# rafaelcgon/2D-GP

Measured on AMD Instinct MI355X. Metric: posterior grid points/sec (fit+predict), N_train=4096, div-free 2D kernel, higher is better.
Workload: dtype f64 (variance GEMM as exact int8 Ozaki-II); 1 GPU; df kernel, N_train=4096, 256x256 grid per GPU, fit+predict (mean+variance); n_train=4096, grid_per_gpu=256x256, points_total=65536, parallelism=grid-sharded x1, factor local, kstar_ahead=False

## Files before the change

2d-gp_amd/csrc/gp2d.hip:

```cpp
#include "common.hpp"
#ifndef GP2D_RELEASE
#error "libgp2d.so is built with -DGP2D_RELEASE=1 (python __graft_entry__.py build)"
#endif
#include "assemble.hpp"
#include "gemm_f64.hpp"
#include "factor.hpp"
#include "predict.hpp"
#include "fields.hpp"
#include "grad.hpp"
#include "postcov.hpp"
#include "predict_host.hpp"
#include "ozaki.hpp"
#include "ozaki_host.hpp"
#include "factor_host.hpp"
#include "lml.hpp"
#include "lml_host.hpp"
#include "dfact.hpp"
#include "order.hpp"
#include "../../include/gp2d.h"

#include <dlfcn.h>

#include <algorithm>
#include <cstdlib>
// ... 1044 lines not shown
  p.diag_add = diag_add;
  p.C = cov; p.ldc = ldc;
  TimedLaunch t(s, 2.0 * (double)ntr * (double)(2 * m) * (double)(2 * m));
  return launch_postcov(p, s);
}

int gp2d_ozaki_nmod(int64_t n) { return ozaki_nmod_for(n); }

size_t gp2d_ozaki_wres_bytes(int64_t n) {
  const int nm = ozaki_nmod_for(n);
  return nm > 0 ? (size_t)nm * (size_t)n * (size_t)n : 0;
}

static int launch_w_res(const double* W, int64_t n, WRows ldw, const OzakiConsts& oc, int8_t* wres,
                        const double* rowscale, hipStream_t s) {
  ozaki_w_res_kernel<<<dim3((unsigned)(n / 64), (unsigned)(n / 256)), 256, 0, s>>>(W, n, ldw, oc, wres, rowscale);
  return check_launch("ozaki_w_res_kernel");
}

static int prepare_args(const gp2d_kernel_t* k, int wbits, int kbits, int64_t n, bool bufs_ok, const int* nmod_out) {
  GP2D_CHECK(validate_ozaki_kernel(k));
  GP2D_CHECK(valid_bits(wbits, kbits));
  GP2D_REQUIRE(n % IBM == 0 && n > 0, "ozaki: n must be a positive multiple of 256");
  GP2D_REQUIRE(bufs_ok, "ozaki: NULL buffer");
  GP2D_REQUIRE(nmod_out != nullptr, "ozaki: nmod_out is NULL");
  return 0;
}

static int prepare_finish(int nmod, const gp2d_kernel_t* k, int pw, int pb, const double* W, int64_t n, WRows wr,
                          int8_t* wres, double* rowscale, bool fused, int* nmod_out, hipStream_t s) {
  OzakiConsts oc;
// ... 105 lines not shown
      const double e = gp2d_ozaki_error_model(kss, vmin, pw, pb);
      if (e <= target && e < best) { best = e; bw = pw; bk = pb; }
    }
    if (bw) {
      *wbits = bw;
      *kbits = bk;
      return 1;
    }
  }
  return 0;
}

static int g_oz_skip = 1;
void gp2d_ozaki_set_skip(int on) { g_oz_skip = on ? 1 : 0; }

size_t gp2d_predict_ozaki_workspace(int64_t n, int64_t chunk) {
  return OzakiWork(n, chunk, ozaki_nmod_for(n), true).total;
}

size_t gp2d_predict_ozaki_workspace_nmod(int64_t n, int64_t chunk, int nmod) {
  if (nmod <= 0 || nmod > ozaki_nmod_for(n)) return 0;
  return std::max(OzakiWork(n, chunk, nmod, true).total, OzakiWork(n, chunk, nmod, false).total);
}

size_t gp2d_predict_ozaki_planes_workspace(int64_t n, int64_t chunk) {
  return OzakiWork(n, chunk, ozaki_nmod_for(n), false).total;
}

struct OzakiChunk {
  int64_t cv, cp, ncols;
  const double* xg;
  dim3 kgrid;
  OzakiChunk(const double* xg0, int64_t m, int64_t c0, int64_t chunk, int64_t ntr_pad, const gp2d_kernel_t* k)
      : cv(std::min<int64_t>(chunk, m - c0)), cp(round_up(cv, IBN)), ncols(2 * cp), xg(xg0 + point_dim(k) * c0),
        kgrid((unsigned)((ntr_pad + OZ_KS_T - 1) / OZ_KS_T), (unsigned)(cp / OZ_KS_P)) {}
};

static int launch_kstar(const OzakiChunk& c, hipStream_t s, const double* xtr, int64_t ntr, int64_t npad,
                        const VecParams& vp, const double* alpha, const OzakiConsts& oc, int8_t* bres, double* pm,
                        uint8_t* flags) {
  if ((uint64_t)(2 * npad) * (uint64_t)c.ncols < (1ull << 31))
    ozaki_kstar_kernel<true><<<c.kgrid, 256, 0, s>>>(xtr, ntr, npad, c.xg, c.cv, c.cp, vp, alpha, oc, bres, pm, flags);
  else
    ozaki_kstar_kernel<false><<<c.kgrid, 256, 0, s>>>(xtr, ntr, npad, c.xg, c.cv, c.cp, vp, alpha, oc, bres, pm, flags);
  return check_launch("ozaki_kstar_kernel");
}

static int predict_ozaki_impl(const int8_t* wres, const double* rowscale, int nmod, int kbits, int64_t n,
                              const double* alpha, const double* xtr, int64_t ntr,
                              int64_t ntr_pad, const double* xg, int64_t m, const gp2d_kernel_t* k, int var_mode,
                              double noise, int compute_var, double* mean, double* var,
                              const int64_t* out_order, int64_t chunk, const OzakiWork& lay, void* work,
                              const KstarBuf* pre, const int8_t* pre_base, hipStream_t s) {
  const auto [bres, cres, pm, P, flags, skip] = lay.at(work);
  OzakiConsts oc;
  GP2D_CHECK(make_ozaki_consts(nmod, k, oc, OZ_PW, ozaki_kbits(kbits)));
  const int nm = oc.nmod;
  GP2D_REQUIRE(n < 131072, "ozaki: the int8 GEMM epilogue needs n < 131072 (N_train < 65536)");
  const int64_t nmseg = (ntr_pad + OZ_KS_T - 1) / OZ_KS_T;
// ... 13 lines not shown
    const size_t bplane = (size_t)ncols * n;
    const bool inline_planes = compute_var && !pre;
    GP2D_CHECK(launch_kstar(c, s, xtr, ntr, ntr_pad, vp, alpha, inline_planes ? oc : oc_mean_only,
                            pre ? nullptr : bres, pm, inline_planes ? flags : nullptr));
    const int nbj = (int)(ncols / IBN), kslabs = (int)(n / IBK);
    const bool use_skip = compute_var && g_oz_skip && kslabs <= (1 << 20);
    int* slist = skip;
    int* scnt = skip + (int64_t)nbj * kslabs;
    if (use_skip) {
      ozaki_slab_list_kernel<<<(unsigned)nbj, 64, 0, s>>>(F, (int)(ntr_pad / OZ_KS_T), nbj, kslabs, slist, scnt);
      GP2D_CHECK(check_launch("ozaki_slab_list_kernel"));
    }
    if (compute_var) {
      const double nv = 2.0 * (double)ntr;
      TimedLaunch timed(s, 2.0 * (double)cv * nv * nv);
      const int zper = (n <= kIgemmZBatchMaxN) ? nm : 1;
      for (int l0 = 0; l0 < nm; l0 += zper) {
        const int nz = std::min(zper, nm - l0);
        IgemmZ zb{(int64_t)n * n, (int64_t)bplane, (int64_t)n * ncols, {}};
        for (int u = 0; u < nz; ++u) zb.m[u] = oc.m[l0 + u];
        constexpr int tbn = 256, nst = I_NSTAGE;
        const dim3 ggrid((unsigned)(ncols / tbn), (unsigned)(n / IBM), (unsigned)nz);
        const int8_t* Al = wres + (size_t)l0 * n * n;
        const int8_t* Bl = B + (size_t)l0 * bplane;
        uint8_t* Cl = cres + (size_t)l0 * n * ncols;
        igemm_nt_mod_kernel<tbn, nst><<<ggrid, 2 * tbn, 0, s>>>(Al, Bl, Cl, n, (int)n, (int)ncols, (int)n, 1, oc.m[l0],
                                                                (int)(cp / IBN), (int)(ntr_pad / IBK),
                                                                use_skip ? slist : nullptr, use_skip ? scnt : nullptr,
                                                                zb);
        GP2D_CHECK(check_launch("igemm_nt_mod_kernel"));
      }
      timed.stop();
      const dim3 cgrid((unsigned)((ncols + OZ_CRT_BCOLS - 1) / OZ_CRT_BCOLS), (unsigned)npseg);
      ozaki_crt_colsq_kernel<<<cgrid, 256, 0, s>>>(cres, n, ncols, oc, rowscale, P);
      GP2D_CHECK(check_launch("ozaki_crt_colsq_kernel"));
    }
    GP2D_CHECK(launch_finalize({pm, nmseg, P, npseg, ncols, cp, cv, c0, m, kss, add, clip, compute_var, mean, var,
                                out_order}, s));
  }
  return 0;
}

static int predict_ozaki_args(const gp2d_kernel_t* k, int64_t n, int64_t ntr_pad, int64_t chunk, int var_mode,
                              bool ptrs_ok, int64_t m, int nmod, int kbits, const OzakiWork& lay, const void* work,
                              size_t work_bytes) {
// ... 503 lines not shown
```

2d-gp_amd/csrc/ozaki.hpp:

```cpp
#pragma once
#include <type_traits>
#include "common.hpp"
#include "assemble.hpp"

namespace gp2d {

constexpr int OZ_MAXMOD = 20;
#ifdef GP2D_OZ_P
#define GP2D_OZ_PW GP2D_OZ_P
#define GP2D_OZ_PB GP2D_OZ_P
#endif
#ifndef GP2D_OZ_PW
#define GP2D_OZ_PW 49
#endif
#ifndef GP2D_OZ_PB
#define GP2D_OZ_PB 45
#endif
constexpr int OZ_PW = GP2D_OZ_PW;
constexpr int OZ_PB = GP2D_OZ_PB;
static_assert(OZ_PW <= 50 && OZ_PB <= 50, "ozaki: the one-part residues need |x| < 2^50");
constexpr int OZ_PW_MAX = 60;
constexpr int OZ_PB_MAX = 50;
constexpr int OZ_SPLIT = 26;
constexpr int OZ_HBITS = 33;
// ... 68 lines not shown
    rowscale[i] = final_scale ? ldexp(M, -si - sB) : (double)si;
    if (l1 != nullptr) l1[i] = sum;
  }
}

__global__ __launch_bounds__(256) void ozaki_rowscale_final_kernel(double* __restrict__ rowscale, int64_t n, double M,
                                                                   int sB) {
  const int64_t i = (int64_t)blockIdx.x * 256 + threadIdx.x;
  if (i < n) rowscale[i] = ldexp(M, -(int)rowscale[i] - sB);
}

__device__ __forceinline__ int ozaki_row_exp(double rowscale_i, const OzakiConsts& oc) {
  return ilogb(oc.M) - ilogb(rowscale_i) - oc.sB;
}

__global__ __launch_bounds__(256) void ozaki_w_res_kernel(const double* __restrict__ W, int64_t n, WRows wr,
                                                          OzakiConsts oc, int8_t* __restrict__ wres,
                                                          const double* __restrict__ rowscale) {
  const int64_t bi = blockIdx.y, ks = blockIdx.x;
  if (ks * 64 >= (bi + 1) * 256) return;
  const int lane = threadIdx.x & 63, wv = threadIdx.x >> 6;
  const int64_t k0 = ks * 64 + 4 * (lane & 15);
  const int64_t plane = n * n;
#pragma unroll 1
  for (int it = 0; it < 16; ++it) {
    const int64_t i = bi * 256 + wv * 64 + it * 4 + (lane >> 4);
    const int si = ozaki_row_exp(rowscale[i], oc);
    const double* w = W + wr.off(i) + k0;
    d2 p0 = {0.0, 0.0}, p1 = {0.0, 0.0};
    if (k0 < wr.len(i, n)) {
      p0 = *reinterpret_cast<const d2*>(w);
      p1 = *reinterpret_cast<const d2*>(w + 2);
    }
    const double v[4] = {p0.x, p0.y, p1.x, p1.y};
    double x[4], xm[4];
#pragma unroll
    for (int u = 0; u < 4; ++u) {
      x[u] = (k0 + u <= i) ? rint(ldexp(v[u], si)) : 0.0;
      xm[u] = x[u] + OZ_MAGIC52;
    }
    int8_t* dst = wres + slab_offset(i, k0, n);
    if (oc.pw <= 50) {
      for (int l = 0; l < oc.nmod; ++l) {
        const double m = oc.md[l], im = oc.inv_m[l];
        uint32_t r[4];
#pragma unroll
        for (int u = 0; u < 4; ++u) r[u] = residue_low_m(x[u], xm[u], m, im);
        *reinterpret_cast<uint32_t*>(dst + (int64_t)l * plane) = pack22(pack2_lo(r[0], r[1]), pack2_lo(r[2], r[3]));
      }
    } else {
      double xh[4], xl[4];
#pragma unroll
      for (int u = 0; u < 4; ++u) {
        xh[u] = rint(ldexp(x[u], -OZ_SPLIT));
        xl[u] = x[u] - ldexp(xh[u], OZ_SPLIT);
      }
      for (int l = 0; l < oc.nmod; ++l) {
        const double m = oc.md[l], im = oc.inv_m[l], c = oc.c26[l];
        uint32_t r[4];
#pragma unroll
        for (int u = 0; u < 4; ++u) {
          const double rh = fma(-m, rint(xh[u] * im), xh[u]), rl = fma(-m, rint(xl[u] * im), xl[u]);
          const double t = fma(rh, c, rl);
          r[u] = residue_low_m(t, t + OZ_MAGIC52, m, im);
        }
        *reinterpret_cast<uint32_t*>(dst + (int64_t)l * plane) = pack22(pack2_lo(r[0], r[1]), pack2_lo(r[2], r[3]));
      }
    }
  }
}

#ifndef GP2D_KS_OCC
#define GP2D_KS_OCC 5
#endif
#ifndef GP2D_KS_PPL
#define GP2D_KS_PPL 2
#endif
constexpr int OZ_KS_T = 64;
constexpr int OZ_KS_P = 64;
constexpr int OZ_KS_PPL = GP2D_KS_PPL;
static_assert(OZ_KS_PPL == 2 || OZ_KS_PPL == 4, "2 or 4 training points per lane");

template <int PPL> struct packed_bytes;
template <> struct packed_bytes<2> { typedef uint16_t type; };
template <> struct packed_bytes<4> { typedef uint32_t type; };

template <bool OFF32>
__global__ __launch_bounds__(256, GP2D_KS_OCC) void ozaki_kstar_kernel(
    const double* __restrict__ xtr, int64_t ntr, int64_t npad, const double* __restrict__ xg, int64_t cv,
    int64_t cp, VecParams vp, const double* __restrict__ alpha, OzakiConsts oc, int8_t* __restrict__ bres,
    double* __restrict__ pm, uint8_t* __restrict__ flags) {
  constexpr int PPL = OZ_KS_PPL, LG = 64 / PPL, RPW = 64 / LG, RPI = 4 * RPW;
  typedef typename packed_bytes<PPL>::type pk_t;
  const int lane = threadIdx.x & 63, wv = threadIdx.x >> 6;
  const int kg = lane % LG, r = lane / LG;
  const int64_t t0 = (int64_t)blockIdx.x * OZ_KS_T + PPL * kg;
  const int64_t n = 2 * npad, ncols = 2 * cp;
  double a1[PPL], a2[PPL], x0[PPL], x1[PPL], x2[PPL];
  bool tv[PPL];
#pragma unroll
  for (int u = 0; u < PPL; ++u) {
    const int64_t t = t0 + u;
// ... 29 lines not shown
        mu += __shfl_xor(mu, o);
        mv += __shfl_xor(mv, o);
      }
      if (kg == 0 && p < cp) {
        pm[(int64_t)blockIdx.x * ncols + p] = mu;
        pm[(int64_t)blockIdx.x * ncols + cp + p] = mv;
      }
    }
    if (p >= cp || t0 >= npad) continue;
    double xi[3][PPL], xm[3][PPL];
#pragma unroll
    for (int u = 0; u < PPL; ++u) {
      xi[0][u] = rint(k11[u] * scale);
      xi[1][u] = rint(k12[u] * scale);
      xi[2][u] = rint(k22[u] * scale);
      nz = nz || xi[0][u] != 0.0 || xi[1][u] != 0.0 || xi[2][u] != 0.0;
#pragma unroll
      for (int e = 0; e < 3; ++e) xm[e][u] = xi[e][u] + OZ_MAGIC52;
    }
    const int64_t o_uu = slab_offset(p, t0, n), o_uv = slab_offset(p, npad + t0, n),
                  o_vv = slab_offset(cp + p, npad + t0, n);
    const int64_t pstride = ncols * n;
    for (int l = 0; l < oc.nmod; ++l) {
      const double m = oc.md[l], im = oc.inv_m[l];
      pk_t pk[3];
#pragma unroll
      for (int e = 0; e < 3; ++e) {
        uint32_t r[PPL];
#pragma unroll
        for (int u = 0; u < PPL; ++u) r[u] = residue_low_m(xi[e][u], xm[e][u], m, im);
        if constexpr (PPL == 2) pk[e] = (pk_t)pack2_lo(r[0], r[1]);
        else pk[e] = (pk_t)pack22(pack2_lo(r[0], r[1]), pack2_lo(r[2], r[3]));
      }
      int8_t* plane = bres + (int64_t)l * pstride;
      if constexpr (OFF32) {
        const __amdgpu_buffer_rsrc_t rs = __builtin_amdgcn_make_buffer_rsrc(plane, (short)0, (int)pstride, 0x00020000);
        if constexpr (PPL == 2) {
          __builtin_amdgcn_raw_buffer_store_b16(pk[0], rs, (int)o_uu, 0, 0);
          __builtin_amdgcn_raw_buffer_store_b16(pk[1], rs, (int)o_uv, 0, 0);
          __builtin_amdgcn_raw_buffer_store_b16(pk[2], rs, (int)o_vv, 0, 0);
        } else {
          __builtin_amdgcn_raw_buffer_store_b32(pk[0], rs, (int)o_uu, 0, 0);
          __builtin_amdgcn_raw_buffer_store_b32(pk[1], rs, (int)o_uv, 0, 0);
          __builtin_amdgcn_raw_buffer_store_b32(pk[2], rs, (int)o_vv, 0, 0);
        }
      } else {
        *reinterpret_cast<pk_t*>(plane + o_uu) = pk[0];
// ... 72 lines not shown
#endif
}

__device__ __forceinline__ int swz16(int row, int chunk) {
  const int q = (row >> 2) & 3;
  const int g = (0x78 >> (2 * q)) & 3;
  return chunk ^ g;
}

template <int P, int W>
__device__ __forceinline__ void vmwait_barrier(std::integral_constant<int, W>) {
  static_assert(P * W < 64, "vmcnt field");
  asm volatile("s_waitcnt vmcnt(%0)\n\ts_waitcnt lgkmcnt(0)\n\ts_barrier" ::"n"(P * W) : "memory");
}

struct IgemmZ {
  int64_t sA, sB, sC;
  int m[OZ_MAXMOD];
};
constexpr int64_t kIgemmZBatchMaxN = 4096;

template <int TBN, int NST>
__global__ __launch_bounds__(TBN * 2, (TBN == 256) ? 1 : 2) void igemm_nt_mod_kernel(
    const int8_t* __restrict__ A, const int8_t* __restrict__ B, uint8_t* __restrict__ C, int64_t ldc, int M, int N,
    int K, int a_lower, int modulus, int alias_rb, int alias_ks, const int* __restrict__ slist,
    const int* __restrict__ scnt, const IgemmZ zb) {
  if (gridDim.z > 1) {
    A += blockIdx.z * zb.sA;
    B += blockIdx.z * zb.sB;
    C += blockIdx.z * zb.sC;
    modulus = zb.m[blockIdx.z];
  }
  static_assert(TBN == 256 || TBN == 128, "tile width");
  static_assert(NST >= 3 && NST <= 5, "ring depth 3..5 (the tail is written out for these)");
  constexpr int NW = TBN / 32;
  constexpr int WC = TBN / 64;
  constexpr int B_OP = TBN * IBK;
  constexpr int STG = I_OP + B_OP;
  constexpr int AP = IBM / NW / 16;
  constexpr int BPW = TBN / NW / 16;
  constexpr int PPW = AP + BPW;
  __shared__ __attribute__((aligned(16))) int8_t smem[NST * STG];
  const int bj = blockIdx.x;
  const int bi = (int)(gridDim.y - 1 - blockIdx.y);
  const int i0 = bi * IBM, j0 = bj * TBN;
  const int jb = j0 / IBN, jr = j0 % IBN;
  const int ke = a_lower ? min(K, i0 + IBM) : K;
  const int tid = threadIdx.x, lane = tid & 63, wid = __builtin_amdgcn_readfirstlane(tid >> 6);
  const int wr = wid / WC, wc = wid % WC;
  const int l16 = lane & 15, lq = lane >> 4;
  const int64_t kslabs = K / IBK;
  const int8_t* Ap = A + (int64_t)bi * kslabs * I_OP;
  const bool alias = jb >= alias_rb;
  const int8_t* Bp = B + (int64_t)jb * kslabs * I_OP + jr * IBK;
  const int8_t* Bq = B + ((int64_t)(alias ? jb - alias_rb : 0) * kslabs + alias_ks) * I_OP + jr * IBK;
  int nsl = ke / IBK;
  const int* sl = nullptr;
  if (slist != nullptr) {
    const int c = scnt[(int64_t)jb * (kslabs / 4 + 1) + ke / IBM];
    if (c == 0 || c >= NST - 1) {
      nsl = c;
      sl = slist + (int64_t)jb * kslabs;
    }
  }

  const int bias = (int)ozaki_acc_bias(K, modulus);
  i4v acc[8][4];
#pragma unroll
  for (int mi = 0; mi < 8; ++mi)
#pragma unroll
    for (int ni = 0; ni < 4; ++ni) acc[mi][ni] = i4v{bias, bias, bias, bias};

  const int drow = lane >> 2, dchunk = lane & 3;
  const int rec = (int)(kslabs * I_OP);
  const __amdgpu_buffer_rsrc_t rA = __builtin_amdgcn_make_buffer_rsrc((void*)Ap, (short)0, rec, 0x00020000);
  const __amdgpu_buffer_rsrc_t rBp = __builtin_amdgcn_make_buffer_rsrc((void*)Bp, (short)0, rec, 0x00020000);
  const __amdgpu_buffer_rsrc_t rBq = __builtin_amdgcn_make_buffer_rsrc((void*)Bq, (short)0, rec, 0x00020000);
  int voA[AP], voB[BPW];
#pragma unroll
  for (int h = 0; h < AP; ++h) {
    const int row = (wid * AP + h) * 16 + drow;
    voA[h] = row * IBK + 16 * swz16(row, dchunk);
  }
#pragma unroll
  for (int h = 0; h < BPW; ++h) {
    const int row = (wid * BPW + h) * 16 + drow;
    voB[h] = row * IBK + 16 * swz16(jr + row, dchunk);
  }
  auto issue = [&](int ks, int st) {
    int8_t* As = smem + st * STG;
    int8_t* Bs = As + I_OP;
    const int so = ks * I_OP;
// ... 24 lines not shown
  auto readb = [&](int st, i4v (&b)[4]) {
    const uint32_t ad = lds_base + st * STG + lane_b;
    asm volatile("ds_read_b128 %0, %1 offset:0" : "=v"(b[0]) : "v"(ad) : "memory");
    asm volatile("ds_read_b128 %0, %1 offset:1024" : "=v"(b[1]) : "v"(ad) : "memory");
    asm volatile("ds_read_b128 %0, %1 offset:2048" : "=v"(b[2]) : "v"(ad) : "memory");
    asm volatile("ds_read_b128 %0, %1 offset:3072" : "=v"(b[3]) : "v"(ad) : "memory");
  };
  auto mfmas = [&](int half, const i4v (&a)[4], const i4v (&b)[4]) {
#pragma unroll
    for (int u = 0; u < 4; ++u)
#pragma unroll
      for (int ni = 0; ni < 4; ++ni)
        acc[4 * half + u][ni] = __builtin_amdgcn_mfma_i32_16x16x64_i8(a[u], b[ni], acc[4 * half + u][ni], 0, 0, 0);
  };
  typedef const __attribute__((address_space(4))) int* const_int_ptr;
  auto slab = [&](int s) -> int { return sl ? ((const_int_ptr)sl)[min(s, nsl - 1)] : s; };
  if (nsl > 0) {
#pragma unroll
    for (int q = 0; q < NST - 1; ++q) issue(slab(q), q);
    int knext = slab(NST - 1);
    vmwait_barrier<PPW>(std::integral_constant<int, NST - 2>{});
    i4v bA[4], a0A[4], bB[4], a0B[4], a1[4];
    readb(0, bA);
    reada(0, 0, a0A);
    __builtin_amdgcn_sched_barrier(0);
    constexpr int LAST = -1;
    auto step = [&](auto dma_c, auto w_c, int s, i4v (&b)[4], i4v (&a0)[4], i4v (&bn)[4], i4v (&a0n)[4]) {
      constexpr bool dma = decltype(dma_c)::value;
      constexpr int w = decltype(w_c)::value;
      const int st = s % NST;
      if constexpr (dma) {
// ... 43 lines not shown
      step(F_{}, std::integral_constant<int, LAST>{}, s + 3, bB, a0B, bA, a0A);
    } else if constexpr (NST == 4) {
      step(F_{}, std::integral_constant<int, 1>{}, s, bA, a0A, bB, a0B);
      step(F_{}, std::integral_constant<int, 0>{}, s + 1, bB, a0B, bA, a0A);
      step(F_{}, std::integral_constant<int, LAST>{}, s + 2, bA, a0A, bB, a0B);
    } else {
      step(F_{}, std::integral_constant<int, 0>{}, s, bA, a0A, bB, a0B);
      step(F_{}, std::integral_constant<int, LAST>{}, s + 1, bB, a0B, bA, a0A);
    }
    asm volatile("s_waitcnt lgkmcnt(0)\n\ts_barrier" ::: "memory");
  }
  uint8_t* T = reinterpret_cast<uint8_t*>(smem);
  constexpr int TP = IBM + 16;
  static_assert(TBN * TP <= NST * STG, "epilogue image fits the ring");
  const OzModConsts mc = ozaki_mod_consts(modulus);
#pragma unroll
  for (int mi = 0; mi < 8; ++mi)
#pragma unroll
    for (int ni = 0; ni < 4; ++ni) {
      uint32_t pk = 0;
#pragma unroll
      for (int u = 0; u < 4; ++u) pk |= ozaki_mod_u32((uint32_t)acc[mi][ni][u], mc) << (8 * u);
      const int rloc = wr * 128 + mi * 16 + 4 * lq;
      const int cloc = wc * 64 + ni * 16 + l16;
      *reinterpret_cast<uint32_t*>(T + cloc * TP + rloc) = pk;
    }
  __syncthreads();
#pragma unroll
  for (int p = 0; p < (IBM * TBN / 16) / (TBN * 2); ++p) {
    const int id = tid + TBN * 2 * p;
    const int cloc = id >> 4, ch = id & 15;
    const i4v v = *reinterpret_cast<const i4v*>(T + cloc * TP + 16 * ch);
    __builtin_nontemporal_store(v, reinterpret_cast<i4v*>(C + (int64_t)(j0 + cloc) * ldc + i0 + 16 * ch));
  }
}

constexpr int OZ_GUARD_RSEG = 256;
__global__ __launch_bounds__(256) void ozaki_guard_colsq_kernel(const double* __restrict__ W, int64_t n, int64_t ldw,
                                                                double* __restrict__ psum, double* __restrict__ pmax) {
  const int64_t c = (int64_t)blockIdx.x * 256 + threadIdx.x, seg = blockIdx.y;
  const int64_t r0 = seg * OZ_GUARD_RSEG, r1 = min<int64_t>(n, r0 + OZ_GUARD_RSEG);
  if (c >= n) return;
  double sq = 0.0, mx = 0.0;
  if (r1 > (int64_t)blockIdx.x * 256) {
#pragma unroll 8
    for (int64_t r = r0; r < r1; ++r) {
      const double w = W[r * ldw + c];
      sq = fma(w, w, sq);
// ... 171 lines not shown
```

2d-gp_amd/csrc/ozaki_host.hpp:

```cpp
#pragma once
#include <algorithm>
#include "ozaki.hpp"

namespace gp2d {

constexpr size_t oz_flag_bytes(int64_t n, int64_t chunk) {
  return (size_t)round_up((round_up(chunk < 1 ? 1 : chunk, IBN) / OZ_KS_P) * (n / 2 / OZ_KS_T), 256);
}
constexpr size_t oz_list_bytes(int64_t n, int64_t chunk) {
  const int64_t nbj = 2 * round_up(chunk < 1 ? 1 : chunk, IBN) / IBN, ks = n / IBK;
  return sizeof(int) * (size_t)(nbj * ks + nbj * (ks / 4 + 1));
}

struct KstarBuf {
  size_t planes, flag_bytes, stride;
  KstarBuf(int64_t n, int64_t chunk, int nmod)
      : planes((size_t)nmod * (size_t)n * (size_t)(2 * round_up(chunk, IBN))), flag_bytes(oz_flag_bytes(n, chunk)),
        stride(planes + flag_bytes) {}
  size_t planes_at(int64_t ci) const { return (size_t)ci * stride; }
  size_t flags_at(int64_t ci) const { return (size_t)ci * stride + planes; }
};

struct OzakiWork {
  size_t bres = 0, cres = 0, pm = 0, P = 0, flags = 0, skip = 0, total = 0;
// ... 6 lines not shown
    cres = bres + (inline_planes ? plane : 0);
    pm = cres + plane;
    P = pm + sizeof(double) * ncols * (inline_planes ? ks_rows : std::max(ks_rows, crt_rows));
    flags = P + sizeof(double) * ncols * crt_rows;
    skip = flags + (inline_planes ? oz_flag_bytes(n, chunk) : 0);
    total = skip + oz_list_bytes(n, chunk);
  }
  struct Ptrs { int8_t* bres; uint8_t* cres; double* pm; double* P; uint8_t* flags; int* skip; };
  Ptrs at(void* work) const {
    char* w = static_cast<char*>(work);
    return {reinterpret_cast<int8_t*>(w + bres), reinterpret_cast<uint8_t*>(w + cres), reinterpret_cast<double*>(w + pm),
            reinterpret_cast<double*>(w + P), reinterpret_cast<uint8_t*>(w + flags), reinterpret_cast<int*>(w + skip)};
  }
};

constexpr bool ozaki_work_ok(int64_t n, int64_t chunk, int nmod) {
  for (int inl = 0; inl < 2; ++inl) {
    const OzakiWork w(n, chunk, nmod, inl);
    if (w.bres != 0 || (w.cres > w.bres) != inl || w.pm <= w.cres || w.P <= w.pm || w.flags <= w.P ||
        w.skip < w.flags || (w.skip > w.flags) != inl || w.total <= w.skip || w.pm % 8 || w.P % 8 || w.skip % 4)
      return false;
  }
  return true;
}
static_assert(ozaki_work_ok(256, 128, 12) && ozaki_work_ok(256, 128, 16) && ozaki_work_ok(8192, 8192, 13),
              "OzakiWork: regions out of order, overlapping or misaligned");

}
```

2d-gp_amd/gp2d/_native.py:

```python
from __future__ import annotations

import ctypes
import os
import threading

_HERE = os.path.dirname(os.path.abspath(__file__))
LIB_PATH = os.environ.get("GP2D_LIB", os.path.join(_HERE, "libgp2d.so"))
ABI_VERSION = 11

FAMILY_VECTOR2D, FAMILY_ARD_RBF, FAMILY_VECTOR_ST = 0, 1, 2
KIND_SCALAR, KIND_DIVFREE, KIND_CURLFREE, KIND_MIXED = 0, 1, 2, 3
VAR_LATENT, VAR_NOISY, VAR_CLIPPED = 0, 1, 2
FIELD_DIVERGENCE, FIELD_VORTICITY = 1, 2
COMM_INT32, COMM_FLOAT64 = 2, 8
COMM_SUM, COMM_MAX, COMM_MIN = 0, 1, 2

EXPORTS = (
    "gp2d_abi_version", "gp2d_build_info", "gp2d_padded_points", "gp2d_block_dim", "gp2d_kernel_diag",
    "gp2d_assemble", "gp2d_factor_sets", "gp2d_factor_warm", "gp2d_factor_set_of", "gp2d_factor_join", "gp2d_potrf_workspace", "gp2d_potrf", "gp2d_trtri_workspace", "gp2d_trtri",
    "gp2d_potrf_inv_workspace", "gp2d_potrf_inv", "gp2d_potrf_batched", "gp2d_trtri_batched_workspace",
    "gp2d_trtri_batched",
    "gp2d_potrs_workspace", "gp2d_potrs_inv", "gp2d_predict_workspace", "gp2d_predict",
    "gp2d_field_prior_var", "gp2d_predict_field_workspace", "gp2d_predict_field",
    "gp2d_grad_prior_cov", "gp2d_predict_grad_workspace", "gp2d_predict_grad",
    "gp2d_predict_cov_workspace", "gp2d_predict_cov",
    "gp2d_ozaki_nmod", "gp2d_ozaki_wres_bytes", "gp2d_ozaki_prepare", "gp2d_ozaki_prepare_async", "gp2d_ozaki_prepare_packed",
    "gp2d_ozaki_guard_workspace", "gp2d_ozaki_guard", "gp2d_ozaki_error_model", "gp2d_ozaki_guard_bits",
    "gp2d_predict_ozaki_workspace", "gp2d_predict_ozaki_workspace_nmod",
    "gp2d_predict_ozaki", "gp2d_ozaki_nmod_apriori", "gp2d_ozaki_kstar_bytes", "gp2d_ozaki_kstar",
    "gp2d_predict_ozaki_planes_workspace", "gp2d_predict_ozaki_planes", "gp2d_ozaki_set_skip", "gp2d_morton_codes",
    "gp2d_morton_sort_workspace", "gp2d_morton_sort", "gp2d_gather_rows", "gp2d_obs_pad", "gp2d_lml", "gp2d_lml_grad_count",
    "gp2d_lml_grad_workspace", "gp2d_lml_grad",
    "gp2d_kernel_grad_count", "gp2d_kernel_grad_workspace", "gp2d_kernel_grad",
    "gp2d_gemm", "gp2d_transpose", "gp2d_comm_id_bytes", "gp2d_comm_unique_id", "gp2d_comm_init",
    "gp2d_comm_destroy", "gp2d_comm_size", "gp2d_bcast", "gp2d_allgather", "gp2d_allreduce", "gp2d_sendrecv",
    "gp2d_stream_create_cumask", "gp2d_stream_destroy", "gp2d_status_flip",
    "gp2d_dfact_sb", "gp2d_dfact_panel_doubles", "gp2d_dfact_workspace", "gp2d_dfact_panel", "gp2d_dfact_update",
    "gp2d_dfact_invstep", "gp2d_dfact_zpart", "gp2d_dfact_zsum", "gp2d_dfact_alpha_workspace", "gp2d_dfact_alpha_blocks",
    "gp2d_assemble_cols", "gp2d_copy2d", "gp2d_zero_upper", "gp2d_pack_lower_doubles", "gp2d_pack_lower",
    "gp2d_timing_enable", "gp2d_timing_read", "gp2d_trace_mark", "gp2d_last_error",
)


class NativeLibraryError(RuntimeError):
    pass
# ... 65 lines not shown
    "gp2d_ozaki_nmod_apriori": (_I, [_I64, _KP, _D, _I, _I]),
    "gp2d_ozaki_prepare_async": (_I, [_P, _I64, _I64, _KP, _D, _I, _I, _P, _P, ctypes.POINTER(_I), _P]),
    "gp2d_ozaki_prepare_packed": (_I, [_P, _I64, _KP, _D, _I, _I, _P, _P, ctypes.POINTER(_I), _P]),
    "gp2d_ozaki_guard_workspace": (_SZ, [_I64]),
    "gp2d_ozaki_guard": (_I, [_P, _I64, _I64, _I64, _I64, _D, _P, _P, _SZ, _P]),
    "gp2d_ozaki_error_model": (_D, [_D, _D, _I, _I]),
    "gp2d_ozaki_guard_bits": (_I, [_D, _D, _D, ctypes.POINTER(_I), ctypes.POINTER(_I)]),
    "gp2d_ozaki_kstar_bytes": (_SZ, [_I64, _I64, _I64, _I]),
    "gp2d_ozaki_kstar": (_I, [_P, _I64, _I64, _P, _I64, _KP, _I, _I, _I64, _P, _SZ, _P]),
    "gp2d_predict_ozaki_planes_workspace": (_SZ, [_I64, _I64]),
    "gp2d_predict_ozaki_planes": (_I, [_P, _P, _I, _I, _I64, _P, _P, _I64, _I64, _P, _I64, _KP, _I, _D, _P, _I, _I,
                                       _P, _P, _P, _I64, _P, _SZ, _P]),
    "gp2d_predict_ozaki_workspace": (_SZ, [_I64, _I64]),
    "gp2d_predict_ozaki_workspace_nmod": (_SZ, [_I64, _I64, _I]),
    "gp2d_ozaki_set_skip": (None, [_I]),
    "gp2d_morton_codes": (_I, [_P, _I64, _I, _P, _P, _P]),
    "gp2d_morton_sort_workspace": (_SZ, [_I64]),
    "gp2d_morton_sort": (_I, [_P, _I64, _I, _P, _P, _P, _SZ, _P]),
    "gp2d_gather_rows": (_I, [_P, _P, _I64, _I64, _P, _P]),
    "gp2d_obs_pad": (_I, [_P, _I64, _I64, _I, _P, _P, _P]),
    "gp2d_predict_ozaki": (_I, [_P, _P, _I, _I, _I64, _P, _P, _I64, _I64, _P, _I64, _KP, _I, _D, _I, _P, _P, _P,
                                _I64, _P, _SZ, _P]),
    "gp2d_lml": (_I, [_P, _I64, _I64, _P, _P, _I64, _P, _P]),
    "gp2d_lml_grad_count": (_I, [_KP]),
    "gp2d_lml_grad_workspace": (_SZ, [_I64]),
    "gp2d_lml_grad": (_I, [_P, _I64, _I64, _P, _P, _I64, _I64, _KP, _P, _P, _SZ, _P]),
    "gp2d_kernel_grad_count": (_I, [_KP]),
    "gp2d_kernel_grad_workspace": (_SZ, [_I64, _I64]),
    "gp2d_kernel_grad": (_I, [_P, _I64, _P, _I64, _KP, _P, _I64, _P, _P, _SZ, _P]),
    "gp2d_gemm": (_I, [_I, _I64, _I64, _I64, _D, _P, _I64, _P, _I64, _D, _P, _I64, _P]),
# ... 105 lines not shown
```

include/gp2d.h:

```cpp
#ifndef GP2D_H
#define GP2D_H

#include <stddef.h>
#include <stdint.h>

#ifdef __cplusplus
extern "C" {
#endif

#define GP2D_ABI_VERSION 11

#define GP2D_FAMILY_VECTOR2D 0
#define GP2D_FAMILY_ARD_RBF  1
#define GP2D_FAMILY_VECTOR_ST 2

#define GP2D_KIND_SCALAR   0
#define GP2D_KIND_DIVFREE  1
#define GP2D_KIND_CURLFREE 2
#define GP2D_KIND_MIXED    3

#define GP2D_VAR_LATENT  0
#define GP2D_VAR_NOISY   1
#define GP2D_VAR_CLIPPED 2

// ... 84 lines not shown
int    gp2d_ozaki_prepare(const double* W, int64_t n, int64_t ldw, const gp2d_kernel_t* k, int wbits, int kbits,
                          int8_t* wres, double* rowscale, int* nmod_out, void* stream);
int    gp2d_ozaki_prepare_async(const double* W, int64_t n, int64_t ldw, const gp2d_kernel_t* k,
                                double diag_add, int wbits, int kbits, int8_t* wres, double* rowscale,
                                int* nmod_out, void* stream);
int    gp2d_ozaki_prepare_packed(const double* packed, int64_t n, const gp2d_kernel_t* k, double diag_add,
                                 int wbits, int kbits, int8_t* wres, double* rowscale, int* nmod_out, void* stream);
size_t gp2d_ozaki_guard_workspace(int64_t n);
int    gp2d_ozaki_guard(const double* W, int64_t n, int64_t ldw, int64_t ntr, int64_t npad, double diag_add,
                        double* stats_dev, void* work, size_t work_bytes, void* stream);
double gp2d_ozaki_error_model(double kss, double vmin, int wbits, int kbits);
int    gp2d_ozaki_guard_bits(double kss, double vmin, double target, int* wbits, int* kbits);
size_t gp2d_predict_ozaki_workspace(int64_t n, int64_t chunk);
size_t gp2d_predict_ozaki_workspace_nmod(int64_t n, int64_t chunk, int nmod);
void   gp2d_ozaki_set_skip(int on);
int    gp2d_morton_codes(const double* pts, int64_t n, int dim, double* bbox, int64_t* codes, void* stream);
size_t gp2d_morton_sort_workspace(int64_t n);
int    gp2d_morton_sort(const double* pts, int64_t n, int dim, double* sorted, int64_t* order, void* work,
                        size_t work_bytes, void* stream);
int    gp2d_gather_rows(const double* src, const int64_t* order, int64_t n, int64_t dim, double* dst,
                        void* stream);
int    gp2d_obs_pad(const double* y, int64_t ntr, int64_t npad, int bd, const int64_t* perm, double* out,
                    void* stream);
int    gp2d_predict_ozaki(const int8_t* wres, const double* rowscale, int nmod, int kbits, int64_t n,
                          const double* alpha, const double* xtr, int64_t ntr, int64_t ntr_pad,
                          const double* xg, int64_t m, const gp2d_kernel_t* k,
                          int var_mode, double noise, int compute_var,
                          double* mean, double* var, const int64_t* out_order, int64_t chunk,
                          void* work, size_t work_bytes, void* stream);
int    gp2d_ozaki_nmod_apriori(int64_t n, const gp2d_kernel_t* k, double diag_add, int wbits, int kbits);
// ... 80 lines not shown
```

Baseline: 1.257 million points/s.

## Compute 2x2 block variance GEMM with three products instead of four

```diff
diff --git a/2d-gp_amd/csrc/gp2d.hip b/2d-gp_amd/csrc/gp2d.hip
--- a/2d-gp_amd/csrc/gp2d.hip
+++ b/2d-gp_amd/csrc/gp2d.hip
@@ -1082,7 +1082,8 @@
 
 static int launch_w_res(const double* W, int64_t n, WRows ldw, const OzakiConsts& oc, int8_t* wres,
                         const double* rowscale, hipStream_t s) {
-  ozaki_w_res_kernel<<<dim3((unsigned)(n / 64), (unsigned)(n / 256)), 256, 0, s>>>(W, n, ldw, oc, wres, rowscale);
+  ozaki_w_res_kernel<<<dim3((unsigned)(n / 64), (unsigned)(n / 256)), 256, 0, s>>>(W, n, ldw, oc, wres, rowscale,
+                                                                                   oz_s_npad(n));
   return check_launch("ozaki_w_res_kernel");
 }
 
@@ -1218,6 +1219,10 @@
 static int g_oz_skip = 1;
 void gp2d_ozaki_set_skip(int on) { g_oz_skip = on ? 1 : 0; }
 
+static int g_oz_three = 1;
+void gp2d_ozaki_set_three_products(int on) { g_oz_three = on ? 1 : 0; }
+static bool ozaki_three(int64_t n) { return g_oz_three && oz_s_npad(n) > 0; }
+
 size_t gp2d_predict_ozaki_workspace(int64_t n, int64_t chunk) {
   return OzakiWork(n, chunk, ozaki_nmod_for(n), true).total;
 }
@@ -1243,10 +1248,19 @@
 static int launch_kstar(const OzakiChunk& c, hipStream_t s, const double* xtr, int64_t ntr, int64_t npad,
                         const VecParams& vp, const double* alpha, const OzakiConsts& oc, int8_t* bres, double* pm,
                         uint8_t* flags) {
-  if ((uint64_t)(2 * npad) * (uint64_t)c.ncols < (1ull << 31))
-    ozaki_kstar_kernel<true><<<c.kgrid, 256, 0, s>>>(xtr, ntr, npad, c.xg, c.cv, c.cp, vp, alpha, oc, bres, pm, flags);
-  else
-    ozaki_kstar_kernel<false><<<c.kgrid, 256, 0, s>>>(xtr, ntr, npad, c.xg, c.cv, c.cp, vp, alpha, oc, bres, pm, flags);
+  const int form = !ozaki_three(2 * npad) ? KS_PLAIN : oc.pb <= 49 ? KS_DIFF_X : KS_DIFF_R;
+  const bool off32 = (uint64_t)(2 * npad) * (uint64_t)c.ncols < (1ull << 31);
+  auto launch = [&](auto off32_c, auto form_c) {
+    ozaki_kstar_kernel<decltype(off32_c)::value, decltype(form_c)::value>
+        <<<c.kgrid, 256, 0, s>>>(xtr, ntr, npad, c.xg, c.cv, c.cp, vp, alpha, oc, bres, pm, flags);
+  };
+  auto pick = [&](auto off32_c) {
+    if (form == KS_PLAIN) launch(off32_c, std::integral_constant<int, KS_PLAIN>{});
+    else if (form == KS_DIFF_X) launch(off32_c, std::integral_constant<int, KS_DIFF_X>{});
+    else launch(off32_c, std::integral_constant<int, KS_DIFF_R>{});
+  };
+  if (off32) pick(std::true_type{});
+  else pick(std::false_type{});
   return check_launch("ozaki_kstar_kernel");
 }
 
@@ -1290,21 +1304,24 @@
     if (compute_var) {
       const double nv = 2.0 * (double)ntr;
       TimedLaunch timed(s, 2.0 * (double)cv * nv * nv);
-      const int zper = (n <= kIgemmZBatchMaxN) ? nm : 1;
+      const bool three = ozaki_three(n);
+      const OzakiProducts prods(n, cp, three);
+      const int zper = (three || n <= kIgemmZBatchMaxN) ? nm : 1;
       for (int l0 = 0; l0 < nm; l0 += zper) {
         const int nz = std::min(zper, nm - l0);
         IgemmZ zb{(int64_t)n * n, (int64_t)bplane, (int64_t)n * ncols, {}};
         for (int u = 0; u < nz; ++u) zb.m[u] = oc.m[l0 + u];
         constexpr int tbn = 256, nst = I_NSTAGE;
-        const dim3 ggrid((unsigned)(ncols / tbn), (unsigned)(n / IBM), (unsigned)nz);
         const int8_t* Al = wres + (size_t)l0 * n * n;
         const int8_t* Bl = B + (size_t)l0 * bplane;
         uint8_t* Cl = cres + (size_t)l0 * n * ncols;
-        igemm_nt_mod_kernel<tbn, nst><<<ggrid, 2 * tbn, 0, s>>>(Al, Bl, Cl, n, (int)n, (int)ncols, (int)n, 1, oc.m[l0],
-                                                                (int)(cp / IBN), (int)(ntr_pad / IBK),
-                                                                use_skip ? slist : nullptr, use_skip ? scnt : nullptr,
-                                                                zb);
-        GP2D_CHECK(check_launch("igemm_nt_mod_kernel"));
+        for (int q = 0; q < prods.count; ++q) {
+          const dim3 ggrid(prods.gx[q], prods.gy[q], (unsigned)nz);
+          igemm_nt_mod_kernel<tbn, nst><<<ggrid, 2 * tbn, 0, s>>>(Al, Bl, Cl, n, kslabs, oc.m[l0], prods.prod[q],
+                                                                  use_skip ? slist : nullptr,
+                                                                  use_skip ? scnt : nullptr, zb);
+          GP2D_CHECK(check_launch("igemm_nt_mod_kernel"));
+        }
       }
       timed.stop();
       const dim3 cgrid((unsigned)((ncols + OZ_CRT_BCOLS - 1) / OZ_CRT_BCOLS), (unsigned)npseg);
diff --git a/2d-gp_amd/csrc/ozaki.hpp b/2d-gp_amd/csrc/ozaki.hpp
--- a/2d-gp_amd/csrc/ozaki.hpp
+++ b/2d-gp_amd/csrc/ozaki.hpp
@@ -1,4 +1,5 @@
 #pragma once
+#include <climits>
 #include <type_traits>
 #include "common.hpp"
 #include "assemble.hpp"
@@ -106,57 +107,86 @@
   return ilogb(oc.M) - ilogb(rowscale_i) - oc.sB;
 }
 
+__device__ __forceinline__ void w_residues4(const double (&x)[4], const OzakiConsts& oc, int l, uint32_t (&r)[4]) {
+  const double m = oc.md[l], im = oc.inv_m[l];
+  if (oc.pw <= 50) {
+#pragma unroll
+    for (int u = 0; u < 4; ++u) r[u] = residue_low_m(x[u], x[u] + OZ_MAGIC52, m, im);
+  } else {
+    const double c = oc.c26[l];
+#pragma unroll
+    for (int u = 0; u < 4; ++u) {
+      const double xh = rint(ldexp(x[u], -OZ_SPLIT));
+      const double xl = x[u] - ldexp(xh, OZ_SPLIT);
+      const double rh = fma(-m, rint(xh * im), xh), rl = fma(-m, rint(xl * im), xl);
+      const double t = fma(rh, c, rl);
+      r[u] = residue_low_m(t, t + OZ_MAGIC52, m, im);
+    }
+  }
+}
+__device__ __forceinline__ uint32_t pack4_lo(const uint32_t (&r)[4]) {
+  return pack22(pack2_lo(r[0], r[1]), pack2_lo(r[2], r[3]));
+}
+__device__ __forceinline__ uint32_t centred_sum(uint32_t a, uint32_t b, int m) {
+  int s = (int)a + (int)b;
+  const int half = m >> 1;
+  s -= (s > half) ? m : 0;
+  s += (s < -half) ? m : 0;
+  return (uint32_t)s;
+}
+
 __global__ __launch_bounds__(256) void ozaki_w_res_kernel(const double* __restrict__ W, int64_t n, WRows wr,
                                                           OzakiConsts oc, int8_t* __restrict__ wres,
-                                                          const double* __restrict__ rowscale) {
+                                                          const double* __restrict__ rowscale, int64_t s_npad) {
   const int64_t bi = blockIdx.y, ks = blockIdx.x;
   if (ks * 64 >= (bi + 1) * 256) return;
+  const int64_t hs = s_npad / 64;
+  const bool fold = hs > 0 && bi * 256 >= s_npad;
+  if (fold && ks >= hs) return;
+  const bool right = fold && (ks + hs) * 64 < (bi + 1) * 256;
   const int lane = threadIdx.x & 63, wv = threadIdx.x >> 6;
   const int64_t k0 = ks * 64 + 4 * (lane & 15);
   const int64_t plane = n * n;
+  auto scaled4 = [&](int64_t i, int64_t kc, int si, double (&x)[4]) {
+    const double* w = W + wr.off(i) + kc;
+    d2 p0 = {0.0, 0.0}, p1 = {0.0, 0.0};
+    if (kc < wr.len(i, n)) {
+      p0 = *reinterpret_cast<const d2*>(w);
+      p1 = *reinterpret_cast<const d2*>(w + 2);
+    }
+    const double v[4] = {p0.x, p0.y, p1.x, p1.y};
+#pragma unroll
+    for (int u = 0; u < 4; ++u) x[u] = (kc + u <= i) ? rint(ldexp(v[u], si)) : 0.0;
+  };
 #pragma unroll 1
   for (int it = 0; it < 16; ++it) {
     const int64_t i = bi * 256 + wv * 64 + it * 4 + (lane >> 4);
     const int si = ozaki_row_exp(rowscale[i], oc);
-    const double* w = W + wr.off(i) + k0;
-    d2 p0 = {0.0, 0.0}, p1 = {0.0, 0.0};
-    if (k0 < wr.len(i, n)) {
-      p0 = *reinterpret_cast<const d2*>(w);
-      p1 = *reinterpret_cast<const d2*>(w + 2);
-    }
-    const double v[4] = {p0.x, p0.y, p1.x, p1.y};
-    double x[4], xm[4];
-#pragma unroll
-    for (int u = 0; u < 4; ++u) {
-      x[u] = (k0 + u <= i) ? rint(ldexp(v[u], si)) : 0.0;
-      xm[u] = x[u] + OZ_MAGIC52;
-    }
+    double x[4];
+    scaled4(i, k0, si, x);
     int8_t* dst = wres + slab_offset(i, k0, n);
-    if (oc.pw <= 50) {
+    if (!fold) {
       for (int l = 0; l < oc.nmod; ++l) {
-        const double m = oc.md[l], im = oc.inv_m[l];
         uint32_t r[4];
-#pragma unroll
-        for (int u = 0; u < 4; ++u) r[u] = residue_low_m(x[u], xm[u], m, im);
-        *reinterpret_cast<uint32_t*>(dst + (int64_t)l * plane) = pack22(pack2_lo(r[0], r[1]), pack2_lo(r[2], r[3]));
+        w_residues4(x, oc, l, r);
+        *reinterpret_cast<uint32_t*>(dst + (int64_t)l * plane) = pack4_lo(r);
       }
     } else {
-      double xh[4], xl[4];
-#pragma unroll
-      for (int u = 0; u < 4; ++u) {
-        xh[u] = rint(ldexp(x[u], -OZ_SPLIT));
-        xl[u] = x[u] - ldexp(xh[u], OZ_SPLIT);
-      }
+      double xr[4] = {0.0, 0.0, 0.0, 0.0};
+      if (right) scaled4(i, s_npad + k0, si, xr);
+      int8_t* dst_r = wres + slab_offset(i, s_npad + k0, n);
+      int8_t* dst_s = wres + slab_offset(i - s_npad, s_npad + k0, n);
       for (int l = 0; l < oc.nmod; ++l) {
-        const double m = oc.md[l], im = oc.inv_m[l], c = oc.c26[l];
-        uint32_t r[4];
-#pragma unroll
-        for (int u = 0; u < 4; ++u) {
-          const double rh = fma(-m, rint(xh[u] * im), xh[u]), rl = fma(-m, rint(xl[u] * im), xl[u]);
-          const double t = fma(rh, c, rl);
-          r[u] = residue_low_m(t, t + OZ_MAGIC52, m, im);
+        uint32_t r[4], q[4] = {0u, 0u, 0u, 0u};
+        w_residues4(x, oc, l, r);
+        *reinterpret_cast<uint32_t*>(dst + (int64_t)l * plane) = pack4_lo(r);
+        if (right) {
+          w_residues4(xr, oc, l, q);
+          *reinterpret_cast<uint32_t*>(dst_r + (int64_t)l * plane) = pack4_lo(q);
         }
-        *reinterpret_cast<uint32_t*>(dst + (int64_t)l * plane) = pack22(pack2_lo(r[0], r[1]), pack2_lo(r[2], r[3]));
+#pragma unroll
+        for (int u = 0; u < 4; ++u) q[u] = centred_sum(r[u], q[u], oc.m[l]);
+        *reinterpret_cast<uint32_t*>(dst_s + (int64_t)l * plane) = pack4_lo(q);
       }
     }
   }
@@ -177,7 +207,8 @@
 template <> struct packed_bytes<2> { typedef uint16_t type; };
 template <> struct packed_bytes<4> { typedef uint32_t type; };
 
-template <bool OFF32>
+enum { KS_PLAIN = 0, KS_DIFF_X = 1, KS_DIFF_R = 2 };
+template <bool OFF32, int FORM>
 __global__ __launch_bounds__(256, GP2D_KS_OCC) void ozaki_kstar_kernel(
     const double* __restrict__ xtr, int64_t ntr, int64_t npad, const double* __restrict__ xg, int64_t cv,
     int64_t cp, VecParams vp, const double* __restrict__ alpha, OzakiConsts oc, int8_t* __restrict__ bres,
@@ -237,7 +268,12 @@
       xi[0][u] = rint(k11[u] * scale);
       xi[1][u] = rint(k12[u] * scale);
       xi[2][u] = rint(k22[u] * scale);
-      nz = nz || xi[0][u] != 0.0 || xi[1][u] != 0.0 || xi[2][u] != 0.0;
+      if constexpr (FORM == KS_DIFF_X) {
+        xi[0][u] -= xi[1][u];
+        xi[2][u] -= xi[1][u];
+      }
+      if constexpr (FORM == KS_DIFF_R) nz = nz || xi[1][u] != 0.0 || xi[0][u] != xi[1][u] || xi[2][u] != xi[1][u];
+      else nz = nz || xi[0][u] != 0.0 || xi[1][u] != 0.0 || xi[2][u] != 0.0;
 #pragma unroll
       for (int e = 0; e < 3; ++e) xm[e][u] = xi[e][u] + OZ_MAGIC52;
     }
@@ -247,13 +283,22 @@
     for (int l = 0; l < oc.nmod; ++l) {
       const double m = oc.md[l], im = oc.inv_m[l];
       pk_t pk[3];
+      uint32_t r[3][PPL];
+#pragma unroll
+      for (int e = 0; e < 3; ++e)
+#pragma unroll
+        for (int u = 0; u < PPL; ++u) r[e][u] = residue_low_m(xi[e][u], xm[e][u], m, im);
+      if constexpr (FORM == KS_DIFF_R) {
+#pragma unroll
+        for (int u = 0; u < PPL; ++u) {
+          r[0][u] = centred_sum(r[0][u], 0u - r[1][u], oc.m[l]);
+          r[2][u] = centred_sum(r[2][u], 0u - r[1][u], oc.m[l]);
+        }
+      }
 #pragma unroll
       for (int e = 0; e < 3; ++e) {
-        uint32_t r[PPL];
-#pragma unroll
-        for (int u = 0; u < PPL; ++u) r[u] = residue_low_m(xi[e][u], xm[e][u], m, im);
-        if constexpr (PPL == 2) pk[e] = (pk_t)pack2_lo(r[0], r[1]);
-        else pk[e] = (pk_t)pack22(pack2_lo(r[0], r[1]), pack2_lo(r[2], r[3]));
+        if constexpr (PPL == 2) pk[e] = (pk_t)pack2_lo(r[e][0], r[e][1]);
+        else pk[e] = (pk_t)pack22(pack2_lo(r[e][0], r[e][1]), pack2_lo(r[e][2], r[e][3]));
       }
       int8_t* plane = bres + (int64_t)l * pstride;
       if constexpr (OFF32) {
@@ -356,6 +401,21 @@
   asm volatile("s_waitcnt vmcnt(%0)\n\ts_waitcnt lgkmcnt(0)\n\ts_barrier" ::"n"(P * W) : "memory");
 }
 
+struct IgemmProd {
+  int bi0;
+  int a_slab0;
+  int a_fold;
+  int a_fold_slab0;
+  int b_rb0;
+  int b_slab0;
+  int alias_rb, alias_ks;
+  int k_bi0, k_cap;
+  int c_col0;
+  int add_col0;
+  static IgemmProd plain(int K, bool lower) {
+    return {0, 0, INT_MAX, 0, 0, 0, INT_MAX, 0, lower ? 0 : -(1 << 20), K, 0, -1};
+  }
+};
 struct IgemmZ {
   int64_t sA, sB, sC;
   int m[OZ_MAXMOD];
@@ -364,9 +424,8 @@
 
 template <int TBN, int NST>
 __global__ __launch_bounds__(TBN * 2, (TBN == 256) ? 1 : 2) void igemm_nt_mod_kernel(
-    const int8_t* __restrict__ A, const int8_t* __restrict__ B, uint8_t* __restrict__ C, int64_t ldc, int M, int N,
-    int K, int a_lower, int modulus, int alias_rb, int alias_ks, const int* __restrict__ slist,
-    const int* __restrict__ scnt, const IgemmZ zb) {
+    const int8_t* __restrict__ A, const int8_t* __restrict__ B, uint8_t* C, int64_t ldc, int kslabs_i, int modulus,
+    const IgemmProd p, const int* __restrict__ slist, const int* __restrict__ scnt, const IgemmZ zb) {
   if (gridDim.z > 1) {
     A += blockIdx.z * zb.sA;
     B += blockIdx.z * zb.sB;
@@ -384,29 +443,33 @@
   constexpr int PPW = AP + BPW;
   __shared__ __attribute__((aligned(16))) int8_t smem[NST * STG];
   const int bj = blockIdx.x;
-  const int bi = (int)(gridDim.y - 1 - blockIdx.y);
+  const int bi = p.bi0 + (int)(gridDim.y - 1 - blockIdx.y);
   const int i0 = bi * IBM, j0 = bj * TBN;
-  const int jb = j0 / IBN, jr = j0 % IBN;
-  const int ke = a_lower ? min(K, i0 + IBM) : K;
+  const int jb = p.b_rb0 + j0 / IBN, jr = j0 % IBN;
+  const int ke = min(p.k_cap, (bi - p.k_bi0 + 1) * IBM);
+  const bool afold = bi >= p.a_fold;
+  const int arb = afold ? bi - p.a_fold : bi, as0 = afold ? p.a_fold_slab0 : p.a_slab0;
   const int tid = threadIdx.x, lane = tid & 63, wid = __builtin_amdgcn_readfirstlane(tid >> 6);
   const int wr = wid / WC, wc = wid % WC;
   const int l16 = lane & 15, lq = lane >> 4;
-  const int64_t kslabs = K / IBK;
-  const int8_t* Ap = A + (int64_t)bi * kslabs * I_OP;
-  const bool alias = jb >= alias_rb;
-  const int8_t* Bp = B + (int64_t)jb * kslabs * I_OP + jr * IBK;
-  const int8_t* Bq = B + ((int64_t)(alias ? jb - alias_rb : 0) * kslabs + alias_ks) * I_OP + jr * IBK;
+  const int64_t kslabs = kslabs_i;
+  const int8_t* Ap = A + ((int64_t)arb * kslabs + as0) * I_OP;
+  const bool alias = jb >= p.alias_rb;
+  const int alias_ks = p.alias_ks;
+  const int8_t* Bp = B + ((int64_t)jb * kslabs + p.b_slab0) * I_OP + jr * IBK;
+  const int8_t* Bq = B + ((int64_t)(alias ? jb - p.alias_rb : 0) * kslabs + alias_ks) * I_OP + jr * IBK;
   int nsl = ke / IBK;
   const int* sl = nullptr;
   if (slist != nullptr) {
-    const int c = scnt[(int64_t)jb * (kslabs / 4 + 1) + ke / IBM];
+    const int* cn = scnt + (int64_t)jb * (kslabs / 4 + 1) + p.b_slab0 / 4;
+    const int c0 = cn[0], c = cn[ke / IBM] - c0;
     if (c == 0 || c >= NST - 1) {
       nsl = c;
-      sl = slist + (int64_t)jb * kslabs;
-    }
-  }
-
-  const int bias = (int)ozaki_acc_bias(K, modulus);
+      sl = slist + (int64_t)jb * kslabs + c0;
+    }
+  }
+
+  const int bias = (int)ozaki_acc_bias(p.k_cap, modulus);
   i4v acc[8][4];
 #pragma unroll
   for (int mi = 0; mi < 8; ++mi)
@@ -414,10 +477,12 @@
     for (int ni = 0; ni < 4; ++ni) acc[mi][ni] = i4v{bias, bias, bias, bias};
 
   const int drow = lane >> 2, dchunk = lane & 3;
-  const int rec = (int)(kslabs * I_OP);
-  const __amdgpu_buffer_rsrc_t rA = __builtin_amdgcn_make_buffer_rsrc((void*)Ap, (short)0, rec, 0x00020000);
-  const __amdgpu_buffer_rsrc_t rBp = __builtin_amdgcn_make_buffer_rsrc((void*)Bp, (short)0, rec, 0x00020000);
-  const __amdgpu_buffer_rsrc_t rBq = __builtin_amdgcn_make_buffer_rsrc((void*)Bq, (short)0, rec, 0x00020000);
+  const __amdgpu_buffer_rsrc_t rA =
+      __builtin_amdgcn_make_buffer_rsrc((void*)Ap, (short)0, (int)((kslabs - as0) * I_OP), 0x00020000);
+  const __amdgpu_buffer_rsrc_t rBp =
+      __builtin_amdgcn_make_buffer_rsrc((void*)Bp, (short)0, (int)((kslabs - p.b_slab0) * I_OP), 0x00020000);
+  const __amdgpu_buffer_rsrc_t rBq =
+      __builtin_amdgcn_make_buffer_rsrc((void*)Bq, (short)0, (int)((kslabs - alias_ks) * I_OP), 0x00020000);
   int voA[AP], voB[BPW];
 #pragma unroll
   for (int h = 0; h < AP; ++h) {
@@ -472,7 +537,8 @@
         acc[4 * half + u][ni] = __builtin_amdgcn_mfma_i32_16x16x64_i8(a[u], b[ni], acc[4 * half + u][ni], 0, 0, 0);
   };
   typedef const __attribute__((address_space(4))) int* const_int_ptr;
-  auto slab = [&](int s) -> int { return sl ? ((const_int_ptr)sl)[min(s, nsl - 1)] : s; };
+  const int b_slab0 = p.b_slab0;
+  auto slab = [&](int s) -> int { return sl ? ((const_int_ptr)sl)[min(s, nsl - 1)] - b_slab0 : s; };
   if (nsl > 0) {
 #pragma unroll
     for (int q = 0; q < NST - 1; ++q) issue(slab(q), q);
@@ -546,24 +612,50 @@
   constexpr int TP = IBM + 16;
   static_assert(TBN * TP <= NST * STG, "epilogue image fits the ring");
   const OzModConsts mc = ozaki_mod_consts(modulus);
-#pragma unroll
-  for (int mi = 0; mi < 8; ++mi)
-#pragma unroll
-    for (int ni = 0; ni < 4; ++ni) {
-      uint32_t pk = 0;
-#pragma unroll
-      for (int u = 0; u < 4; ++u) pk |= ozaki_mod_u32((uint32_t)acc[mi][ni][u], mc) << (8 * u);
-      const int rloc = wr * 128 + mi * 16 + 4 * lq;
-      const int cloc = wc * 64 + ni * 16 + l16;
-      *reinterpret_cast<uint32_t*>(T + cloc * TP + rloc) = pk;
-    }
+  constexpr int NP = (IBM * TBN / 16) / (TBN * 2);
+  auto epilogue = [&](auto add_c) {
+    constexpr bool add = decltype(add_c)::value;
+    if constexpr (add) {
+      const uint8_t* Cp = C + (int64_t)(p.add_col0 + j0) * ldc + i0;
+      i4v pv[NP];
+#pragma unroll
+      for (int q = 0; q < NP; ++q) {
+        const int id = tid + TBN * 2 * q;
+        pv[q] = __builtin_nontemporal_load(reinterpret_cast<const i4v*>(Cp + (int64_t)(id >> 4) * ldc + 16 * (id & 15)));
+      }
+#pragma unroll
+      for (int q = 0; q < NP; ++q) {
+        const int id = tid + TBN * 2 * q;
+        *reinterpret_cast<i4v*>(T + (id >> 4) * TP + 16 * (id & 15)) = pv[q];
+      }
+      __syncthreads();
+    }
+#pragma unroll
+    for (int mi = 0; mi < 8; ++mi)
+#pragma unroll
+      for (int ni = 0; ni < 4; ++ni) {
+        const int rloc = wr * 128 + mi * 16 + 4 * lq;
+        const int cloc = wc * 64 + ni * 16 + l16;
+        uint32_t* t = reinterpret_cast<uint32_t*>(T + cloc * TP + rloc);
+        uint32_t prior = 0;
+        if constexpr (add) prior = *t;
+        uint32_t pk = 0;
+#pragma unroll
+        for (int u = 0; u < 4; ++u)
+          pk |= ozaki_mod_u32((uint32_t)acc[mi][ni][u] + ((prior >> (8 * u)) & 0xffu), mc) << (8 * u);
+        *t = pk;
+      }
+  };
+  if (p.add_col0 >= 0) epilogue(std::true_type{});
+  else epilogue(std::false_type{});
   __syncthreads();
-#pragma unroll
-  for (int p = 0; p < (IBM * TBN / 16) / (TBN * 2); ++p) {
-    const int id = tid + TBN * 2 * p;
+  uint8_t* Cc = C + (int64_t)(p.c_col0 + j0) * ldc + i0;
+#pragma unroll
+  for (int q = 0; q < NP; ++q) {
+    const int id = tid + TBN * 2 * q;
     const int cloc = id >> 4, ch = id & 15;
     const i4v v = *reinterpret_cast<const i4v*>(T + cloc * TP + 16 * ch);
-    __builtin_nontemporal_store(v, reinterpret_cast<i4v*>(C + (int64_t)(j0 + cloc) * ldc + i0 + 16 * ch));
+    __builtin_nontemporal_store(v, reinterpret_cast<i4v*>(Cc + (int64_t)cloc * ldc + 16 * ch));
   }
 }
 
diff --git a/2d-gp_amd/csrc/ozaki_host.hpp b/2d-gp_amd/csrc/ozaki_host.hpp
--- a/2d-gp_amd/csrc/ozaki_host.hpp
+++ b/2d-gp_amd/csrc/ozaki_host.hpp
@@ -44,6 +44,34 @@
   }
 };
 
+constexpr int64_t oz_s_npad(int64_t n) { return (n > 0 && n % (2 * IBM) == 0) ? n / 2 : 0; }
+
+struct OzakiProducts {
+  int count;
+  IgemmProd prod[3];
+  unsigned gx[3], gy[3];
+  OzakiProducts(int64_t n, int64_t cp, bool three) {
+    const int nb = (int)(n / IBM), nbh = (int)(cp / IBN), hs = (int)(n / 2 / IBK);
+    if (!three) {
+      count = 1;
+      prod[0] = IgemmProd::plain((int)n, true);
+      prod[0].alias_rb = nbh;
+      prod[0].alias_ks = hs;
+      gx[0] = 2u * nbh;
+      gy[0] = (unsigned)nb;
+      return;
+    }
+    const int nb2 = nb / 2, npad = (int)(n / 2), vcol = (int)cp;
+    count = 3;
+    prod[0] = {0,   0,      nb2,    hs,          0,    hs,     INT_MAX, 0,       0,    npad, vcol,  -1};
+    prod[1] = {0,   0,      INT_MAX, 0,          0,    0,      INT_MAX, 0,       0,    npad, 0,     vcol};
+    prod[2] = {nb2, hs,     INT_MAX, 0,          nbh,  hs,     INT_MAX, 0,       nb2,  npad, vcol,  vcol};
+    gx[0] = gx[1] = gx[2] = (unsigned)nbh;
+    gy[0] = gy[1] = (unsigned)nb;
+    gy[2] = (unsigned)nb2;
+  }
+};
+
 constexpr bool ozaki_work_ok(int64_t n, int64_t chunk, int nmod) {
   for (int inl = 0; inl < 2; ++inl) {
     const OzakiWork w(n, chunk, nmod, inl);
diff --git a/2d-gp_amd/gp2d/_native.py b/2d-gp_amd/gp2d/_native.py
--- a/2d-gp_amd/gp2d/_native.py
+++ b/2d-gp_amd/gp2d/_native.py
@@ -28,7 +28,8 @@
     "gp2d_ozaki_guard_workspace", "gp2d_ozaki_guard", "gp2d_ozaki_error_model", "gp2d_ozaki_guard_bits",
     "gp2d_predict_ozaki_workspace", "gp2d_predict_ozaki_workspace_nmod",
     "gp2d_predict_ozaki", "gp2d_ozaki_nmod_apriori", "gp2d_ozaki_kstar_bytes", "gp2d_ozaki_kstar",
-    "gp2d_predict_ozaki_planes_workspace", "gp2d_predict_ozaki_planes", "gp2d_ozaki_set_skip", "gp2d_morton_codes",
+    "gp2d_predict_ozaki_planes_workspace", "gp2d_predict_ozaki_planes", "gp2d_ozaki_set_skip", "gp2d_ozaki_set_three_products",
+    "gp2d_morton_codes",
     "gp2d_morton_sort_workspace", "gp2d_morton_sort", "gp2d_gather_rows", "gp2d_obs_pad", "gp2d_lml", "gp2d_lml_grad_count",
     "gp2d_lml_grad_workspace", "gp2d_lml_grad",
     "gp2d_kernel_grad_count", "gp2d_kernel_grad_workspace", "gp2d_kernel_grad",
@@ -124,6 +125,7 @@
     "gp2d_predict_ozaki_workspace": (_SZ, [_I64, _I64]),
     "gp2d_predict_ozaki_workspace_nmod": (_SZ, [_I64, _I64, _I]),
     "gp2d_ozaki_set_skip": (None, [_I]),
+    "gp2d_ozaki_set_three_products": (None, [_I]),
     "gp2d_morton_codes": (_I, [_P, _I64, _I, _P, _P, _P]),
     "gp2d_morton_sort_workspace": (_SZ, [_I64]),
     "gp2d_morton_sort": (_I, [_P, _I64, _I, _P, _P, _P, _SZ, _P]),
diff --git a/include/gp2d.h b/include/gp2d.h
--- a/include/gp2d.h
+++ b/include/gp2d.h
@@ -122,6 +122,7 @@
 size_t gp2d_predict_ozaki_workspace(int64_t n, int64_t chunk);
 size_t gp2d_predict_ozaki_workspace_nmod(int64_t n, int64_t chunk, int nmod);
 void   gp2d_ozaki_set_skip(int on);
+void   gp2d_ozaki_set_three_products(int on);
 int    gp2d_morton_codes(const double* pts, int64_t n, int dim, double* bbox, int64_t* codes, void* stream);
 size_t gp2d_morton_sort_workspace(int64_t n);
 int    gp2d_morton_sort(const double* pts, int64_t n, int dim, double* sorted, int64_t* order, void* work,
```

Result: faster. 1.315 million points/s (median of 6 runs) (+4.6%).
